# TtesseractT/Synthetic-Audio-Detection

Measured on AMD Instinct MI355X. Metric: 4s@32kHz segments/sec end-to-end (mel+ResNet+ensemble), 1/2/4/8 MI355X, higher is better.
Workload: dtype bf16; 1 GPU; end-to-end inference: B int16 4 s segments resident in HBM -> mel front end -> ResNet-18@512x512 -> 6 binary heads -> merge (+RCCL all-gather of logits); heads=6, distinct_backbones=1, micro_batch=2048, parallelism=dp1, frontend_overlapped=True

## Files before the change

### synthetic-audio-detection_amd/csrc/api.hip

```cpp
#include <math.h>
#include <stdlib.h>
#include <string.h>

#include <mutex>
#include <string>
#include <vector>

#include "common.hpp"
#include "kernels.hpp"

namespace sad {

static thread_local std::string g_err;
void set_error(const std::string& msg) { g_err = msg; }

struct ConvSpec {
  int cin, cout, k, stride, pad;
};
static std::vector<ConvSpec> resnet18_specs() {
  std::vector<ConvSpec> v;
  v.push_back({3, 64, 7, 2, 3});
  int inp = 64;
  const int planes[4] = {64, 128, 256, 512};
  for (int li = 0; li < 4; ++li) {
// ... 334 lines not shown
}

extern "C" int sad_profile_end(int32_t variant, double* total_ms, int64_t* launches, double* flops) {
  SAD_REQUIRE(total_ms && launches && flops, "null outputs");
  std::lock_guard<std::mutex> lk(g_prof_mu);
  g_prof_on = false;
  double ms = 0.0, fl = 0.0;
  int64_t n = 0;
  for (auto& r : g_prof) {
    if (variant == 0 || r.variant == variant) {
      SAD_CHECK_HIP(hipEventSynchronize(r.e1));
      float t = 0.f;
      SAD_CHECK_HIP(hipEventElapsedTime(&t, r.e0, r.e1));
      ms += t;
      fl += r.flops;
      n += r.kernels;
    }
    (void)hipEventDestroy(r.e0);
    (void)hipEventDestroy(r.e1);
  }
  g_prof.clear();
  *total_ms = ms;
  *launches = n;
  *flops = fl;
  return SAD_OK;
}

static int run_blocks(const sad_backbone_plan* p, size_t b0, size_t b1, int64_t n, void** in, void** alt, void* tmp,
                      int& H, int& C, hipStream_t s, float* pool_out = nullptr, bool* pooled = nullptr) {
  int rc;
  void* bufA = *in;
  void* bufB = *alt;
  void* bufT = tmp;
  const int64_t mb = n;
  {
    for (size_t bi = b0; bi < b1; ++bi) {
      const DevBlock& blk = p->blocks[bi];
      const int Ho = H / blk.stride;
      if (p->dtype == SAD_BF16 && blk.stride == 1 && blk.cout == 64 && C == 64 && blk.cin == 64 && H % 16 == 0 &&
          l1_fused()) {
        L1BlockArgs f{};
        f.x = (const u16*)bufA;
        f.out = (u16*)bufB;
        f.N = (int)mb;
        f.H = f.W = H;
        f.w1 = (const u16*)blk.w1;
        f.w1_ld = 9 * 64;
        f.b1 = blk.b1;
        f.w2 = (const u16*)blk.w2;
        f.w2_ld = 9 * 64 + blk.cin_sc;
        f.b2 = blk.b2;
        if ((rc = timed_l1block(f, s, 2.0 * 2.0 * mb * H * H * 64 * 576.0))) return rc;
        std::swap(bufA, bufB);
        continue;
      }
      BlockConvArgs a{};
      a.in0 = bufA;
      a.in0_pstride = C;
      a.N = (int)mb;
      a.H = a.W = H;
      a.Cin = C;
      a.KH = a.KW = 3;
      a.stride = blk.stride;
      a.pad = 1;
      a.wt = blk.w1;
      a.bias = blk.b1;
      a.out = bufT;
      a.out_pstride = blk.cout;
      a.Ho = a.Wo = Ho;
      a.Cout = blk.cout;
      a.relu = 1;
      a.M = mb * Ho * Ho;
      if ((rc = timed_block_conv(a, p->dtype, s, 2.0 * a.M * a.Cout * 9.0 * C))) return rc;
      BlockConvArgs b2 = a;
      b2.in0 = bufT;
      b2.in0_pstride = blk.cout;
      b2.H = b2.W = Ho;
      b2.Cin = blk.cout;
      b2.stride = 1;
      b2.wt_ld = 9 * blk.cout + blk.cin_sc;
      if ((p->dtype == SAD_BF16 || p->dtype == SAD_BF16X3) && blk.stride == 1 && Ho % 16 == 0 &&
          (blk.cout <= 64 || (blk.cout <= 128 && layer2_halo() && !(p->dtype == SAD_BF16 && layer2_v31()) &&
                            !(p->dtype == SAD_BF16X3 && x3_layer2_v31())))) {
        b2.res = bufA;
        b2.res_pstride = C;
      } else {
        b2.in1 = bufA;
        b2.in1_pstride = C;
        b2.H1 = b2.W1 = H;
        b2.Cin1 = C;
        b2.ss1 = blk.stride;
      }
      b2.wt = blk.w2;
      b2.bias = blk.b2;
      b2.out = bufB;
      if (pool_out && bi + 1 == b1 && block_conv_can_pool(b2, p->dtype)) {
        b2.pool_out = pool_out;
        b2.out = nullptr;
        *pooled = true;
      }
      const double fl2 = 2.0 * b2.M * b2.Cout * (9.0 * blk.cout + (blk.stride != 1 ? (double)C : 0.0));
      if ((rc = timed_block_conv(b2, p->dtype, s, fl2))) return rc;
      std::swap(bufA, bufB);
      H = Ho;
      C = blk.cout;
    }
  }
  *in = bufA;
  *alt = bufB;
  return SAD_OK;
}

static int front_sub_batch(int dtype) {
  static int v = [] {
    const char* e = getenv("SAD_FRONT_MB");
    return e ? atoi(e) : -1;
  }();
  if (v >= 0) return v;
  return dtype == SAD_BF16 && l1_fused() ? 256 : dtype == SAD_BF16X3 ? 64 : 32;
}

static int run_chunk(const sad_backbone_plan* p, const float* map, const float* img, int64_t mb, float* feats,
                     void* layer4_out, char* ws, hipStream_t s, const float* img3 = nullptr) {
  const size_t ab = act_bytes(p, mb);
  void* bufA = ws;
  void* bufB = ws + ab;
  void* bufT = ws + 2 * ab;
  void* bufD = ws + 3 * ab;
  int rc;
  int H = 128, C = 64;
  bool pooled = false;
  if (p->block_path) {
    const size_t es = p->dtype == SAD_BF16 ? 2 : 4;
    const int64_t f = front_sub_batch(p->dtype) > 0 ? std::min<int64_t>(front_sub_batch(p->dtype), mb) : mb;
    const size_t l1_elems = 128 * 128 * 64;
    for (int64_t i = 0; i < mb; i += f) {
      const int64_t n = std::min(f, mb - i);
      void* a0 = bufA;
      void* a1 = bufB;
      StemArgs st{map ? map + i * p->mh * p->mw : nullptr, img ? img + i * 512 * 512 : nullptr, p->mh, p->mw,
                  p->stem_w, p->stem_b, a0, n, img3 ? img3 + i * 3 * 512 * 512 : nullptr, p->stem_w3};
      if ((rc = launch_stem(st, p->dtype, s))) return rc;
      H = 128;
      C = 64;
      if ((rc = run_blocks(p, 0, 1, n, &a0, &a1, bufT, H, C, s))) return rc;
      void* slot = (char*)bufD + (size_t)i * l1_elems * es;
      void* dst = slot;
      void* src = a0;
      if ((rc = run_blocks(p, 1, 2, n, &src, &dst, bufT, H, C, s))) return rc;
      if (src != slot) {
        set_error("internal: layer1 output not in its bufD slot");
        return SAD_ERR_STATE;
      }
    }
    void* a0 = bufD;
    void* a1 = bufA;
    if ((rc = run_blocks(p, 2, p->blocks.size(), mb, &a0, &a1, bufB, H, C, s, layer4_out ? nullptr : feats,
                         &pooled)))
      return rc;
    bufA = a0;
  } else {
    StemArgs st{map, img, p->mh, p->mw, p->stem_w, p->stem_b, bufA, mb, img3, p->stem_w3};
    if ((rc = launch_stem(st, p->dtype, s))) return rc;
  }
  size_t ci = 0;
  for (int li = 0; li < 4 && !p->block_path; ++li) {
// ... 403 lines not shown
```

### synthetic-audio-detection_amd/csrc/block.hip

```cpp
#include <stdio.h>
#include <stdlib.h>

#include <algorithm>
#include <atomic>
#include <type_traits>
#include <vector>

#include "common.hpp"
#include "igemm.hpp"
#include "kernels.hpp"

#ifndef SAD_STAMPS
#define SAD_STAMPS 0
#endif

namespace sad {

#define SAD_STAMP(slot)                                                                          \
  do {                                                                                           \
    if constexpr (SAD_STAMPS) {                                                                  \
      if (stamp_on) {                                                                            \
        __builtin_amdgcn_sched_barrier(0);                                                       \
        uint64_t t_;                                                                             \
        asm volatile("s_memtime %0\n\ts_waitcnt lgkmcnt(0)" : "=s"(t_)::"memory");              \
// ... 526 lines not shown
  g = std::max<int64_t>(n_tc, g / n_tc * n_tc);
  const int64_t nk = (int64_t)a.KH * a.KW * a.Cin * sizeof(T) / 128 + (a.in1 ? a.Cin1 * sizeof(T) / 128 : 0);
  SAD_REQUIRE(a.M + BP < (1ll << 31) && (tiles_p / (g / n_tc) + 1) * nk < (1ll << 31),
              "block conv: too many pixels for one launch (lower the micro-batch)");
  if constexpr (ST_OK) {
    if (a.st_part) {
      *a.st_rows = (int)(g / n_tc);
      hipLaunchKernelGGL((block_conv_kernel<T, WC, WP, TC, TP, S, OCC, false, X3, true>), dim3((unsigned)g),
                         dim3(64 * WC * WP), smem, s, a);
      SAD_CHECK_HIP(hipGetLastError());
      return SAD_OK;
    }
  }
  if constexpr (RES_OK) {
    if (a.res) {
      hipLaunchKernelGGL((block_conv_kernel<T, WC, WP, TC, TP, S, OCC, true, X3, false, X4>), dim3((unsigned)g),
                         dim3(64 * WC * WP), smem, s, a);
      SAD_CHECK_HIP(hipGetLastError());
      return SAD_OK;
    }
  }
  hipLaunchKernelGGL((block_conv_kernel<T, WC, WP, TC, TP, S, OCC, false, X3, false, X4>), dim3((unsigned)g),
                     dim3(64 * WC * WP),
                     smem, s, a);
  SAD_CHECK_HIP(hipGetLastError());
  return SAD_OK;
}

template <typename T, bool X3 = false>
static int launch_block_v(const BlockConvArgs& a, int v, hipStream_t s) {
  switch (v) {
    case 9: return launch_block_t<T, 1, 4, 4, 4, 2, 2, false, X3>(a, s);
    case 10: return launch_block_t<T, 2, 2, 4, 4, 2, 2, false, X3>(a, s);
    case 11: return launch_block_t<T, 1, 4, 4, 4, 3, 1, false, X3>(a, s);
    case 12: return launch_block_t<T, 2, 2, 4, 4, 3, 1, false, X3>(a, s);
    case 13: return launch_block_t<T, 2, 4, 8, 4, 2, 1, true, X3, sizeof(T) == 2 && !X3>(a, s);
    case 14: return launch_block_t<T, 2, 4, 4, 4, 2, 1, false, X3>(a, s);
    case 15: return launch_block_t<T, 2, 4, 4, 4, 3, 1, false, X3, sizeof(T) == 2 && !X3>(a, s);
    case 16: return launch_block_t<T, 1, 8, 4, 4, 2, 1, false, X3>(a, s);
    case 17: return launch_block_t<T, 2, 2, 8, 4, 2, 1, false, X3>(a, s);
    case 18: return launch_block_t<T, 2, 2, 4, 8, 2, 1, false, X3>(a, s);
    case 19: return launch_block_t<T, 1, 8, 8, 4, 2, 1, false, X3>(a, s);
  }
  set_error("unknown block-conv variant");
  return SAD_ERR_ARG;
}
static int launch_block_x4(const BlockConvArgs& a, int v, hipStream_t s) {
  switch (v) {
    case 9: return launch_block_t<u16, 1, 4, 4, 4, 2, 2, false, true, false, true>(a, s);
    case 13: return launch_block_t<u16, 2, 4, 8, 4, 2, 1, true, true, false, true>(a, s);
    case 15: return launch_block_t<u16, 2, 4, 4, 4, 3, 1, false, true, false, true>(a, s);
  }
  set_error("four-product split-bf16 convs run on the implicit-GEMM variants 9, 13, 15");
  return SAD_ERR_ARG;
}

int launch_halo_v(const BlockConvArgs& a, int v, hipStream_t s, bool x3 = false);
int launch_halo256(const BlockConvArgs& a, hipStream_t s, bool x3);
int launch_halo256r(const BlockConvArgs& a, hipStream_t s, bool x3);
bool halo256_ok(const BlockConvArgs& a);
int launch_halo_rw(const BlockConvArgs& a, hipStream_t s);
int launch_l2conv(const BlockConvArgs& a, hipStream_t s, bool x3 = false);
int launch_halo256s2(const BlockConvArgs& a, hipStream_t s);
bool halo256s2_ok(const BlockConvArgs& a);
int launch_halo_rw_x3(const BlockConvArgs& a, hipStream_t s);
int launch_l2s2conv(const BlockConvArgs& a, hipStream_t s);
int launch_halo256rs2(const BlockConvArgs& a, hipStream_t s, bool x3);
bool halo256rs2_ok(const BlockConvArgs& a);

static bool halo_ok(const BlockConvArgs& a, int dtype) {
  return (dtype == SAD_BF16 || dtype == SAD_BF16X3) && a.KH == 3 && a.KW == 3 && a.stride == 1 && a.pad == 1 &&
         !a.in1 && a.Cin % (dtype == SAD_BF16X3 ? 32 : 64) == 0 && a.Cout % 64 == 0 && a.W % 16 == 0 &&
         a.H % 16 == 0;
}
bool layer2_v31() {
  static const bool v = [] {
    const char* e = getenv("SAD_L2_V31");
    return e ? atoi(e) != 0 : false;
  }();
  return v;
}
static bool halo31_ok(const BlockConvArgs& a) {
  return a.KH == 3 && a.KW == 3 && a.stride == 1 && a.pad == 1 && a.Cout % 128 == 0 && a.H % 16 == 0 &&
         a.W % 16 == 0 && a.Ho == a.H && a.Wo == a.W && !a.res && !a.st_part && a.Cin % 64 == 0 &&
         (!a.in1 || a.Cin1 % 64 == 0) && (!a.pool_out || (a.H == 16 && a.W == 16 && a.Cout % 256 == 0));
}
bool x3_layer2_v31() {
  static const bool v = [] {
    const char* e = getenv("SAD_X3_L2_V31");
    return e ? atoi(e) != 0 : true;
  }();
  return v;
}
static bool l2_rw() {
  static const bool v = [] {
    const char* e = getenv("SAD_L2_RW");
    return e ? atoi(e) != 0 : true;
  }();
  return v;
}
static bool l2_ds_rw() {
  static const bool v = [] {
    const char* e = getenv("SAD_L2_DS_RW");
    return e ? atoi(e) != 0 : true;
  }();
  return v;
}
static bool l2conv_ds_ok(const BlockConvArgs& a) {
  return a.KH == 3 && a.KW == 3 && a.stride == 1 && a.pad == 1 && a.Cin == 128 && a.Cout == 128 && a.H % 16 == 0 &&
         a.W % 16 == 0 && a.Ho == a.H && a.Wo == a.W && a.in1 && a.Cin1 == 64 && a.ss1 == 2 && a.H1 == 2 * a.H &&
         a.W1 == 2 * a.W && !a.res && !a.pool_out && !a.st_part;
}
static int s2_patch() {
  static const int v = [] {
    const char* e = getenv("SAD_S2_PATCH");
    return e ? atoi(e) : 2;
  }();
  return v;
}
static int x3_s2_variant() {
  static const int v = [] {
    const char* e = getenv("SAD_X3_S2");
    return e ? atoi(e) : 44;
  }();
  return v;
}
static bool l2s2_rw() {
  static const bool v = [] {
    const char* e = getenv("SAD_L2S2_RW");
    return e ? atoi(e) != 0 : true;
  }();
  return v;
}
static bool l2s2_ok(const BlockConvArgs& a) {
  return a.KH == 3 && a.KW == 3 && a.stride == 2 && a.pad == 1 && a.Cin == 64 && a.Cout == 128 && a.Ho % 16 == 0 &&
         a.Wo % 16 == 0 && a.H == 2 * a.Ho && a.W == 2 * a.Wo && !a.in1 && !a.res && !a.pool_out;
}
bool layer2_halo() {
  static const bool v = [] {
    const char* e = getenv("SAD_L2_HALO");
    return e ? atoi(e) != 0 : true;
  }();
  return v;
}
static int c128_variant() {
  static const int v = [] {
    const char* e = getenv("SAD_C128_VARIANT");
    return e ? atoi(e) : 15;
  }();
  return v;
}
static int halo_c128_variant() {
  static const int v = [] {
    const char* e = getenv("SAD_HALO_C128");
    return e ? atoi(e) : 20;
  }();
  return v;
}
static int x3_l1_variant() {
  static const int v = [] {
    const char* e = getenv("SAD_X3_L1");
    return e ? atoi(e) : 42;
  }();
  return v;
}
static bool x3_rw() {
  static const bool v = [] {
    const char* e = getenv("SAD_X3_RW");
    return e ? atoi(e) != 0 : true;
  }();
  return v;
}
static int x3_halo256_variant() {
  static const int v = [] {
    const char* e = getenv("SAD_X3_HALO256");
    return e ? atoi(e) : 30;
  }();
  return v;
}
static int halo256_mode() {
  static const int v = [] {
    const char* e = getenv("SAD_HALO256");
    return e ? atoi(e) : 2;
  }();
  return v;
}
static int block_device_cus() {
  static int cus[64] = {};
  int dev = 0;
  if (hipGetDevice(&dev) != hipSuccess || dev < 0 || dev >= 64) return 256;
  if (!cus[dev]) {
    int c = 0;
    if (hipDeviceGetAttribute(&c, hipDeviceAttributeMultiprocessorCount, dev) != hipSuccess || c <= 0) c = 256;
    cus[dev] = c;
  }
  return cus[dev];
}
int default_block_variant(const BlockConvArgs& a, int dtype) {
  if (dtype == SAD_BF16X3) {
    if (halo_ok(a, dtype) && a.Cin == 64 && a.Cout == 64 && x3_l1_variant() == 42) return 42;
    if (halo_ok(a, dtype) && a.Cin == 64 && a.Cout == 64 && x3_rw()) return 26;
    if (x3_layer2_v31() && a.Cout == 128 && halo31_ok(a)) return 31;
    if (halo256_mode() != 0 && (halo256_mode() == 1 || x3_halo256_variant() == 30) && halo256_ok(a)) return 30;
    if (halo256_mode() == 2 && x3_halo256_variant() == 31 && a.Cout % 256 == 0 && halo31_ok(a)) return 31;
    if (x3_s2_variant() == 44 && halo256rs2_ok(a) && a.Cout % 256 == 0) return 44;
    return halo_ok(a, dtype) && a.Cout <= 128 ? 20 : (a.Cout % 256 == 0 ? 13 : (a.Cout % 128 == 0 ? c128_variant() : 9));
  }
  if (halo_ok(a, dtype) && a.Cin == 64 && a.Cout == 64) return 25;
  if (dtype == SAD_BF16 && l2_rw() && halo_ok(a, dtype) && a.Cin == 128 && a.Cout == 128 && !a.st_part) return 41;
  if (dtype == SAD_BF16 && l2_ds_rw() && l2conv_ds_ok(a)) return 41;
  if (dtype == SAD_BF16 && layer2_v31() && a.Cout == 128 && halo31_ok(a)) return 31;
  if (halo_ok(a, dtype) && (a.res || (a.Cout <= 128 && layer2_halo())))
    return a.Cout == 128 && !a.res && halo_c128_variant() == 22 ? 22 : 20;
  if (dtype == SAD_BF16 && halo256_mode() != 0 && halo256_ok(a)) return halo256_mode() == 2 ? 31 : 30;
  if (dtype == SAD_BF16 && l2s2_rw() && l2s2_ok(a)) return 43;
  if (dtype == SAD_BF16 && s2_patch() == 2 && halo256rs2_ok(a)) return 44;
  if (dtype == SAD_BF16 && s2_patch() == 1 && halo256s2_ok(a)) return 32;
  return gemm_block_variant(a);
}
int gemm_block_variant(const BlockConvArgs& a) {
  if (a.Cout % 256 == 0)
    return a.res || (a.M + 255) / 256 * (a.Cout / 256) >= block_device_cus() ? 13 : 15;
  return a.Cout % 128 == 0 ? c128_variant() : 9;
}
static int pool_tile(int v) {
  switch (v) {
    case 13: case 14: case 15: case 30: case 31: return 256;
    case 16: return 512;
  }
  return 0;
}
bool block_conv_can_pool(const BlockConvArgs& a, int dtype) {
  const int v = default_block_variant(a, dtype);
  const int bp = pool_tile(v);
  return bp > 0 && a.Ho * a.Wo == bp && !a.res && a.M % bp == 0 && (v != 31 || a.Cout % 256 == 0);
}
static bool variant_fits(int v, int cout) {
  if (v == 26 || v == 42) return cout == 64;
  if (v == 30) return cout % 256 == 0;
  if (v == 31 || v == 32 || v == 44) return cout % 128 == 0;
  const int bc[] = {0, 0, 0, 0, 0, 0, 0, 0, 0, 64, 128, 64, 128, 256, 128, 128, 64, 256, 128, 128};
  if (v == 20 || v == 21) return cout % 64 == 0;
  if (v == 22) return cout % 128 == 0;
  if (v == 25) return cout == 64;
  if (v == 41 || v == 43) return cout == 128;
  return v >= 9 && v <= 19 && cout % bc[v] == 0;
}

#if SAD_STAMPS
constexpr size_t kStampWords = SAD_CLOCK_BASE + 4 * SAD_CLOCK_WGS;
static bool stamp_this_launch(int which) {
  static const int every = [] {
    const char* e = getenv("SAD_STAMP_EVERY");
    return e ? std::max(1, atoi(e)) : 1;
  }();
  static long count[2] = {0, 0};
  return count[which]++ % every == every - 1;
}
static int stamp_report(const BlockConvArgs& a, hipStream_t s) {
  std::vector<uint64_t> h(kStampWords);
  SAD_CHECK_HIP(hipStreamSynchronize(s));
  SAD_CHECK_HIP(hipMemcpy(h.data(), a.stamps, h.size() * 8, hipMemcpyDeviceToHost));
  {
    std::vector<double> clk, dur, xcd[8];
    uint64_t r0 = ~0ull, r0max = 0, r1min = ~0ull, r1 = 0;
    for (int g = 0; g < SAD_CLOCK_WGS; ++g) {
      const uint64_t* c = &h[SAD_CLOCK_BASE + 4 * g];
      if (!c[0] || !c[2] || c[3] <= c[1]) continue;
      clk.push_back((double)(c[2] - c[0]) / (double)(c[3] - c[1]) * 100.0);
      xcd[g % 8].push_back(clk.back());
      dur.push_back((double)(c[3] - c[1]) / 100.0);
      r0 = std::min(r0, c[1]); r0max = std::max(r0max, c[1]);
      r1min = std::min(r1min, c[3]); r1 = std::max(r1, c[3]);
    }
    if (!clk.empty()) {
      std::sort(clk.begin(), clk.end());
      std::sort(dur.begin(), dur.end());
      fprintf(stderr, "clock M=%lld Cout=%d: %zu workgroups, in-kernel clock median %.0f MHz (min %.0f, max %.0f); "
              "span %.1f us, workgroup time median %.1f us (min %.1f, max %.1f), starts spread %.1f us, "
              "ends spread %.1f us\n", (long long)a.M, a.Cout, clk.size(), clk[clk.size() / 2], clk.front(),
              clk.back(), (r1 - r0) / 100.0, dur[dur.size() / 2], dur.front(), dur.back(), (r0max - r0) / 100.0,
              (r1 - r1min) / 100.0);
      fprintf(stderr, "clock per XCD (median MHz):");
      for (auto& x : xcd) {
        if (x.empty()) continue;
        std::sort(x.begin(), x.end());
        fprintf(stderr, " %.0f", x[x.size() / 2]);
      }
      fprintf(stderr, "\n");
    }
  }
  for (int w = 0; w < 2; ++w) {
    double ph[4] = {0, 0, 0, 0};
    int n = 0;
    for (int g = a.N <= 64 ? 1 : 8; g + 1 < 1024; ++g) {
      const uint64_t* t = &h[w * 4096 + g * 4];
      const uint64_t t0n = h[w * 4096 + (g + 1) * 4];
      if (!t[0] || !t[3] || !t0n || t0n < t[3]) break;
      ph[0] += (double)(t[1] - t[0]);
      ph[1] += (double)(t[2] - t[1]);
      ph[2] += (double)(t[3] - t[2]);
      ph[3] += (double)(t0n - t[3]);
      ++n;
    }
    if (n)
      fprintf(stderr, "stamps M=%lld Cout=%d K=%d wave %d: %d steps, cycles/step phases 0-1 %.0f | 1-2 %.0f | "
              "2-3 %.0f | 3-next %.0f | total %.0f\n", (long long)a.M, a.Cout, a.KH * a.KW * a.Cin, w, n,
              ph[0] / n, ph[1] / n, ph[2] / n, ph[3] / n, (ph[0] + ph[1] + ph[2] + ph[3]) / n);
  }
  return SAD_OK;
}
#endif

static thread_local int64_t g_block_conv_kernels = 0;
int64_t block_conv_kernel_launches() { return g_block_conv_kernels; }

int launch_block_conv(const BlockConvArgs& a_in, int dtype, hipStream_t s, int variant) {
  SAD_REQUIRE(dtype == SAD_F32 || dtype == SAD_BF16 || dtype == SAD_BF16X3, "dtype");
// ... 150 lines not shown
```

### synthetic-audio-detection_amd/csrc/halo256r.hip

```cpp
#include "common.hpp"
#include "igemm.hpp"
#include "kernels.hpp"
#include "rwconv.hpp"

namespace sad {

namespace h31 {
constexpr int NW = 8, TC = 2;
constexpr int TW = 16, TH = 16, PW = TW + 2, PR = PW * (TH + 2);
constexpr int NDP = (PR + 7) / 8;
constexpr int SCR = PW * TH;
constexpr int NDS = SCR / 8;
constexpr int PATCH = NDP * 1024;
constexpr int ROWB = PW * 128;
constexpr int SMEM = 2 * PATCH;
constexpr int BAD = 0x7FFFFFF0;
constexpr uint64_t KEY = 0xd92dad912240ull;
static_assert(SMEM <= 160 * 1024, "LDS budget");
}

__device__ __forceinline__ int h31_key(int px) { return (int)((h31::KEY >> (3 * px)) & 7); }

typedef unsigned int h31_v4 __attribute__((ext_vector_type(4)));
typedef __bf16 h31_bf2 __attribute__((ext_vector_type(2)));
typedef float h31_f2 __attribute__((ext_vector_type(2)));
__device__ __forceinline__ uint32_t h31_pk(float lo, float hi) {
  return __builtin_bit_cast(uint32_t, __builtin_convertvector((h31_f2){lo, hi}, h31_bf2));
}
__device__ __forceinline__ uint32_t h31_relu2(uint32_t x) {
  uint32_t r;
  asm("v_pk_max_i16 %0, %1, 0" : "=v"(r) : "v"(x));
  return r;
}

template <int BC, bool POOL, bool X3 = false>
__global__ __launch_bounds__(512, 1) void halo256r_kernel(BlockConvArgs a) {
  using namespace h31;
  constexpr int NCG = BC / 32, NPG = NW / NCG, TP = 16 / NPG;
  static_assert(NCG * NPG == NW && (!POOL || NPG == 1), "wave split");
  extern __shared__ __attribute__((aligned(16))) char smem[];
  const int tid = threadIdx.x, lane = tid & 63;
  const int wave = __builtin_amdgcn_readfirstlane(tid >> 6);
  const int fr = lane & 15, fg = lane >> 4;
  const int n_tc = a.Cout / BC;
  const int w = xcd_remap(blockIdx.x, gridDim.x);
  const int tc = w % n_tc;
  const int gp = gridDim.x / n_tc, wi = w / n_tc;
  const int tiles_x = a.W / TW, tiles_img = tiles_x * (a.H / TH);
  const int tiles_p = a.N * tiles_img;
  const int tp_begin = (int)((int64_t)wi * tiles_p / gp), tp_end = (int)((int64_t)(wi + 1) * tiles_p / gp);
  const int c0 = tc * BC;
  if (tp_begin >= tp_end) return;
  const int cgrp = wave % NCG, pgrp = wave / NCG;
  const int cw = c0 + cgrp * 16 * TC;
  const int r0w = pgrp * TP;

  const int cinb = a.Cin * 2;
  const int nc0 = cinb / 128;
  const int nk1 = a.in1 ? a.Cin1 * 2 / 128 : 0;
  const int nch = nc0 + nk1;

  const __amdgpu_buffer_rsrc_t r0 =
      __builtin_amdgcn_make_buffer_rsrc((void*)a.in0, (short)0, (int)a.in0_bytes, 0x00020000);
  const __amdgpu_buffer_rsrc_t r1 =
      __builtin_amdgcn_make_buffer_rsrc((void*)(a.in1 ? a.in1 : a.in0), (short)0, (int)a.in1_bytes, 0x00020000);
  const __amdgpu_buffer_rsrc_t rw =
      __builtin_amdgcn_make_buffer_rsrc((void*)a.wt, (short)0, (int)a.wt_bytes, 0x00020000);
  const int ps0 = (int)a.in0_pstride * 2, ps1 = (int)a.in1_pstride * 2;
  const unsigned lds0 = (unsigned)(uintptr_t)(__attribute__((address_space(3))) char*)smem;
  const int lrow = lane >> 3;
  const int ab = a.ablate;

  const int wrow = a.wt_ld * 2;
  const int wlane = (cw + fr) * wrow + fg * 16;
  auto load_w = [&](int kb, h31_v4 (&wv)[TC][2]) __attribute__((always_inline)) {
#pragma unroll
    for (int i = 0; i < TC; ++i)
#pragma unroll
      for (int h = 0; h < 2; ++h)
        wv[i][h] = __builtin_amdgcn_raw_buffer_load_b128(rw, wlane + i * 16 * wrow + kb + h * 64, 0, 0);
  };
  auto kb_of = [&](int c, int tap) __attribute__((always_inline)) {
    return c < nc0 ? tap * cinb + c * 128 : 9 * cinb + (c - nc0) * 128;
  };

  struct TileO {
    int b, oy0, ox0;
    bool ok;
  };
  auto tile_o = [&](int t) __attribute__((always_inline)) {
    const int tt = __builtin_amdgcn_readfirstlane(t);
    const int b = tt / tiles_img, rem = tt - b * tiles_img;
    const int ty = rem / tiles_x;
    return TileO{b, ty * TH, (rem - ty * tiles_x) * TW, tt < tp_end};
  };
  auto issue_patch = [&](const TileO& to, int c, int buf, int k_only) __attribute__((always_inline)) {
    if (!to.ok) return;
    const int b = to.b, oy0 = to.oy0, ox0 = to.ox0;
    int lr;
    asm volatile("v_mov_b32 %0, %1" : "=v"(lr) : "v"(lrow));
    const unsigned dst = lds0 + buf * PATCH;
    if (c < nc0) {
      const int base = ((b * a.H + oy0 - 1) * a.W + ox0 - 1) * ps0 + c * 128;
#pragma unroll
      for (int k = 0; k < (NDP + NW - 1) / NW; ++k) {
        const int q = wave + NW * k;
        if ((k_only < 0 || k == k_only) && q < NDP) {
          const int s = 8 * q + lr, py = s / PW, px = s - py * PW;
          const int iy = oy0 - 1 + py, ix = ox0 - 1 + px;
          const int off = (s < PR && (unsigned)iy < (unsigned)a.H && (unsigned)ix < (unsigned)a.W)
                              ? base + (py * a.W + px) * ps0 + (((lane & 7) ^ h31_key(px)) << 4)
                              : BAD;
          dma16_m0(r0, off, dst + q * 1024);
        }
      }
    } else {
      const int base = ((b * a.H1 + oy0 * a.ss1) * a.W1 + ox0 * a.ss1) * ps1 + (c - nc0) * 128;
#pragma unroll
      for (int k = 0; k < (NDS + NW - 1) / NW; ++k) {
        const int q = wave + NW * k;
        if ((k_only < 0 || k == k_only) && q < NDS) {
          const int s = 8 * q + lr, ty = s / PW, tx = s - ty * PW;
          const int off = tx < TW ? base + (ty * a.W1 + tx) * (a.ss1 * ps1) + (((lane & 7) ^ h31_key(tx)) << 4)
                                  : BAD;
          dma16_m0(r1, off, dst + q * 1024);
        }
      }
    }
  };

  issue_patch(tile_o(tp_begin), 0, 0, -1);
  f32x4 biasv[TC];
#pragma unroll
  for (int i = 0; i < TC; ++i) biasv[i] = *(const f32x4*)(a.bias + cw + i * 16 + fg * 4);
  h31_v4 wcur[TC][2], wnxt[TC][2];
  load_w(0, wnxt);

  f32x4 acc[TC][TP];
#pragma unroll
  for (int i = 0; i < TC; ++i)
#pragma unroll
    for (int j = 0; j < TP; ++j) acc[i][j] = biasv[i];

  auto take_w = [&]() __attribute__((always_inline)) {
#pragma unroll
    for (int i = 0; i < TC; ++i)
#pragma unroll
      for (int h = 0; h < 2; ++h) wcur[i][h] = wnxt[i][h];
  };

  auto step = [&](int pbuf, int ky, int kx) __attribute__((always_inline)) {
    const int pbase = pbuf * PATCH + (ky + r0w) * ROWB;
    const int o0 = (kx + fr) * 128 + ((fg ^ h31_key(kx + fr)) << 4);
    const int o1 = (kx + fr) * 128 + (((fg + 4) ^ h31_key(kx + fr)) << 4);
    const char* pb0 = smem + pbase + o0;
    const char* pb1 = smem + pbase + o1;
    auto half = [&](auto hc) __attribute__((always_inline)) {
      constexpr int h = decltype(hc)::value;
      constexpr int NM = X3 && h == 0 ? 2 : 1;
      const char* pb = h ? pb1 : pb0;
      uint4 bf[TP];
#pragma unroll
      for (int j = 0; j < TP; ++j) bf[j] = *(const uint4*)(pb + j * ROWB);
#pragma unroll
      for (int j = 0; j < TP; ++j)
#pragma unroll
        for (int m = 0; m < NM; ++m)
#pragma unroll
          for (int i = 0; i < TC; ++i)
            mfma_chunk<u16>(__builtin_bit_cast(uint4, wcur[i][X3 ? m : h]), bf[j], acc[i][j]);
      __builtin_amdgcn_sched_group_barrier(0x100, 4, 0);
#pragma unroll
      for (int j = 0; j < TP - 4; ++j) {
        __builtin_amdgcn_sched_group_barrier(0x008, NM * TC, 0);
        __builtin_amdgcn_sched_group_barrier(0x100, 1, 0);
      }
      __builtin_amdgcn_sched_group_barrier(0x008, 4 * NM * TC, 0);
    };
    half(std::integral_constant<int, 0>{});
    half(std::integral_constant<int, 1>{});
  };

  auto epilogue = [&](int t) __attribute__((always_inline)) {
    const int b = t / tiles_img, rem = t - b * tiles_img;
    const int oy0 = (rem / tiles_x) * TH, ox0 = (rem - (rem / tiles_x) * tiles_x) * TW;
    if constexpr (POOL) {
#pragma unroll
      for (int i = 0; i < TC; ++i) {
        float ps[4];
#pragma unroll
        for (int r = 0; r < 4; ++r) {
          float v = 0.f;
#pragma unroll
          for (int j = 0; j < TP; ++j) v += fmaxf(acc[i][j][r], 0.f);
          ps[r] = row16_sum(v);
        }
        if (fr == 0)
          *(float4*)(a.pool_out + (int64_t)b * a.Cout + cw + i * 16 + fg * 4) =
              make_float4(ps[0] * (1.f / 256), ps[1] * (1.f / 256), ps[2] * (1.f / 256), ps[3] * (1.f / 256));
      }
    } else {
      u16* __restrict__ out = (u16*)a.out;
#pragma unroll
      for (int j = 0; j < TP; j += 2) {
        const int64_t px = (int64_t)(b * a.H + oy0 + r0w + j + (fg & 1)) * a.W + ox0 + fr;
#pragma unroll
        for (int i = 0; i < TC; ++i) {
          if constexpr (X3) {
            float v[2][4];
#pragma unroll
            for (int r = 0; r < 4; ++r) {
              v[0][r] = a.relu ? fmaxf(acc[i][j][r], 0.f) : acc[i][j][r];
              v[1][r] = a.relu ? fmaxf(acc[i][j + 1][r], 0.f) : acc[i][j + 1][r];
            }
            uint32_t qh[4], ql[4];
#pragma unroll
            for (int e = 0; e < 4; ++e) {
              const float x0 = v[e >> 1][2 * (e & 1)], x1 = v[e >> 1][2 * (e & 1) + 1];
              qh[e] = h31_pk(x0, x1);
              ql[e] = h31_pk(x0 - __uint_as_float(qh[e] << 16), x1 - __uint_as_float(qh[e] & 0xFFFF0000u));
            }
#pragma unroll
            for (int e = 0; e < 2; ++e) {
              const auto rh = __builtin_amdgcn_permlane16_swap(qh[e], qh[e + 2], false, false);
              qh[e] = rh[0];
              qh[e + 2] = rh[1];
              const auto rl = __builtin_amdgcn_permlane16_swap(ql[e], ql[e + 2], false, false);
              ql[e] = rl[0];
              ql[e + 2] = rl[1];
            }
            u16* op = out + px * a.out_pstride + 2 * cw + i * 16 + (fg >> 1) * 8;
            *(uint4*)op = make_uint4(qh[0], qh[1], qh[2], qh[3]);
            *(uint4*)(op + 32) = make_uint4(ql[0], ql[1], ql[2], ql[3]);
            continue;
          }
          const int co = cw + i * 16 + (fg >> 1) * 8;
          uint32_t q[4] = {h31_pk(acc[i][j][0], acc[i][j][1]), h31_pk(acc[i][j][2], acc[i][j][3]),
                           h31_pk(acc[i][j + 1][0], acc[i][j + 1][1]), h31_pk(acc[i][j + 1][2], acc[i][j + 1][3])};
          if (a.relu)
#pragma unroll
            for (int e = 0; e < 4; ++e) q[e] = h31_relu2(q[e]);
#pragma unroll
          for (int e = 0; e < 2; ++e) {
            const auto r = __builtin_amdgcn_permlane16_swap(q[e], q[e + 2], false, false);
            q[e] = r[0];
            q[e + 2] = r[1];
          }
          if (ab & 128) {
            asm volatile("" ::"v"(q[0]), "v"(q[1]), "v"(q[2]), "v"(q[3]));
          } else {
            *(uint4*)(out + px * a.out_pstride + co) = make_uint4(q[0], q[1], q[2], q[3]);
          }
        }
      }
    }
#pragma unroll
    for (int i = 0; i < TC; ++i)
#pragma unroll
      for (int j = 0; j < TP; ++j) acc[i][j] = biasv[i];
  };

  int u = 0;
  bool post_epi = false;
  for (int t = tp_begin; t < tp_end; ++t) {
    for (int c = 0; c < nch; ++c) {
      const bool sc = c >= nc0;
      const int nsteps = sc ? 1 : 9;
      const int nt = c + 1 < nch ? t : t + 1, ncn = c + 1 < nch ? c + 1 : 0;
      const TileO nto = tile_o(nt);
      const int pbuf = u & 1;
      for (int tap = 0; tap < nsteps; ++tap) {
        if (tap == 0) {
          if (post_epi)
            asm volatile("s_waitcnt vmcnt(%0)" ::"n"(POOL ? 0 : (X3 ? 2 : 1) * TC * TP / 2) : "memory");
          else
            asm volatile("s_waitcnt vmcnt(0)" ::: "memory");
          post_epi = false;
          __builtin_amdgcn_s_barrier();
          asm volatile("" ::: "memory");
        }
        take_w();
        if (!(ab & 1)) {
          const int kbn = tap + 1 < nsteps ? kb_of(c, tap + 1) : kb_of(ncn, 0);
          if (!(ab & 4)) load_w(kbn, wnxt);
          if (ab & 2) {
          } else if (sc) {
            issue_patch(nto, ncn, pbuf ^ 1, -1);
          } else if (tap >= 1 && tap <= 6) {
            issue_patch(nto, ncn, pbuf ^ 1, tap - 1);
          }
        }
        const int ky = sc ? 0 : tap / 3, kx = sc ? 0 : tap - 3 * (tap / 3);
        step(pbuf, ky, kx);
      }
      ++u;
    }
    if (!(ab & 8)) epilogue(t);
    post_epi = true;
  }
  asm volatile("s_waitcnt vmcnt(0)" ::: "memory");
}

template <int BC, bool POOL, bool X3>
static int launch_halo256r_t(const BlockConvArgs& a, hipStream_t s) {
  using namespace h31;
  static bool attr = false;
  if (!attr) {
    (void)hipFuncSetAttribute((const void*)halo256r_kernel<BC, POOL, X3>,
                              hipFuncAttributeMaxDynamicSharedMemorySize, SMEM);
    attr = true;
  }
  const int n_tc = a.Cout / BC;
  const int64_t tiles_p = (int64_t)a.N * (a.H / TH) * (a.W / TW);
  int64_t g = std::min<int64_t>(tiles_p * n_tc, 256);
  g = std::max<int64_t>(n_tc, g / n_tc * n_tc);
  hipLaunchKernelGGL((halo256r_kernel<BC, POOL, X3>), dim3((unsigned)g), dim3(512), SMEM, s, a);
  SAD_CHECK_HIP(hipGetLastError());
  return SAD_OK;
}

int launch_halo256r(const BlockConvArgs& a, hipStream_t s, bool x3) {
  SAD_REQUIRE(a.KH == 3 && a.KW == 3 && a.stride == 1 && a.pad == 1, "variant 31: 3x3, stride 1, pad 1");
  SAD_REQUIRE(!a.res && !a.st_part, "variant 31: no epilogue residual / fused statistics (shortcut as in1)");
  SAD_REQUIRE(a.Cout % 128 == 0, "variant 31: Cout must be a multiple of 128");
  SAD_REQUIRE(a.H % 16 == 0 && a.W % 16 == 0 && a.Ho == a.H && a.Wo == a.W, "variant 31: image must tile by 16 x 16");
  SAD_REQUIRE((a.Cin * 2) % 128 == 0 && (!a.in1 || (a.Cin1 * 2) % 128 == 0), "variant 31: whole 128-B chunks");
  SAD_REQUIRE(!a.in1 || ((a.Ho - 1) * a.ss1 < a.H1 && (a.Wo - 1) * a.ss1 < a.W1), "variant 31: shortcut source");
  SAD_REQUIRE(a.wt_ld >= 9 * a.Cin + (a.in1 ? a.Cin1 : 0) && (a.wt_ld * 2) % 16 == 0, "variant 31: weight rows");
  SAD_REQUIRE(a.out_pstride % 8 == 0 && a.in0_pstride % 8 == 0 && (!a.in1 || a.in1_pstride % 8 == 0),
              "variant 31: pixel strides");
  SAD_REQUIRE(a.out || a.pool_out, "null output");
  SAD_REQUIRE(a.M == (int64_t)a.N * a.H * a.W, "variant 31: M = N H W");
  if (a.pool_out) {
    SAD_REQUIRE(a.H == 16 && a.W == 16 && a.Cout % 256 == 0,
                "variant 31 fused average pool: a 16 x 16 tile must be one image, Cout % 256");
    return x3 ? launch_halo256r_t<256, true, true>(a, s) : launch_halo256r_t<256, true, false>(a, s);
  }
  if (x3)
    return a.Cout % 256 == 0 ? launch_halo256r_t<256, false, true>(a, s) : launch_halo256r_t<128, false, true>(a, s);
  return a.Cout % 256 == 0 ? launch_halo256r_t<256, false, false>(a, s) : launch_halo256r_t<128, false, false>(a, s);
}

}
```

### synthetic-audio-detection_amd/csrc/kernels.hpp

```cpp
#pragma once
#include <vector>

#include "common.hpp"

namespace sad {

#define SAD_CLOCK_BASE 8192
#define SAD_CLOCK_WGS 4096
#define SAD_CLOCK_STAMP(slot)                                                                      \
  do {                                                                                             \
    if constexpr (SAD_STAMPS) {                                                                    \
      if (a.stamps && wave == 0 && blockIdx.x < SAD_CLOCK_WGS) {                                   \
        const uint64_t t_ = __builtin_amdgcn_s_memtime();                                          \
        const uint64_t r_ = __builtin_amdgcn_s_memrealtime();                                      \
        if (lane == 0) {                                                                           \
          a.stamps[SAD_CLOCK_BASE + 4 * blockIdx.x + 2 * (slot)] = t_;                             \
          a.stamps[SAD_CLOCK_BASE + 4 * blockIdx.x + 2 * (slot) + 1] = r_;                         \
        }                                                                                          \
      }                                                                                            \
    }                                                                                              \
  } while (0)

struct ConvArgs {
  const void* in;
// ... 5 lines not shown
  int64_t res_pstride;
  void* out;
  int64_t out_pstride;
  int Ho, Wo, Cout, KH, KW, stride, pad;
  int relu;
  int64_t M;
  int64_t in_bytes;
  int64_t wt_bytes;
  int groups;
  int64_t in_gstride, wt_gstride, bias_gstride, out_gstride;
};

struct BlockConvArgs {
  const void* in0;
  int64_t in0_pstride;
  int N, H, W, Cin, KH, KW, stride, pad;
  const void* in1;
  int64_t in1_pstride;
  int H1, W1, Cin1, ss1;
  const void* wt;
  int wt_ld;
  const float* bias;
  const void* res;
  int64_t res_pstride;
  void* out;
  int64_t out_pstride;
  int Ho, Wo, Cout, relu;
  int64_t M;
  int64_t in0_bytes, in1_bytes, wt_bytes, res_bytes;
  int64_t out_bytes;
  int ablate;
  float* pool_out;
  uint64_t* stamps;
  float* st_part;
  int* st_rows;
  int x4;
};

struct L1BlockArgs {
  const u16* x;
  u16* out;
  int N, H, W;
  const u16* w1;
  int w1_ld;
  const float* b1;
  const u16* w2;
  int w2_ld;
  const float* b2;
  int64_t x_bytes;
  int ablate;
  uint64_t* stamps;
};
int launch_l1block(const L1BlockArgs& a, hipStream_t s);
int64_t block_conv_kernel_launches();
bool l1_fused();

struct StemArgs {
  const float* map;
  const float* img;
  int mh, mw;
  const void* w;
  const float* bias;
  void* out;
  int64_t B;
  const float* img3;
  const float* w3;
  const u16* img16;
  float* part;
  int x4;
};

int launch_conv(const ConvArgs& a, int dtype, hipStream_t s, int variant = 0);
int default_conv_variant(const ConvArgs& a);
int launch_stem(const StemArgs& a, int dtype, hipStream_t s);
int launch_stem_train(const StemArgs& a, hipStream_t s);
constexpr int STEM_TRAIN_PARTS = 16;
int launch_block_conv(const BlockConvArgs& a, int dtype, hipStream_t s, int variant = 0);
int default_block_variant(const BlockConvArgs& a, int dtype);
int gemm_block_variant(const BlockConvArgs& a);
bool layer2_halo();
bool x3_layer2_v31();
bool layer2_v31();
bool block_conv_can_pool(const BlockConvArgs& a, int dtype);
int launch_col2im(const float* dcol, int64_t N, int H, int W, int C, int k, int stride, int pad, int Ho, int Wo,
                  int accumulate, void* dx, int dtype, hipStream_t s);
int launch_avgpool(const void* in, int64_t B, int hw, int c, float* out, int dtype, hipStream_t s);
int launch_heads_final(const float* y2, int64_t B, int n_heads, const float* w3, const float* b3,
                       float* logits, float* merged, hipStream_t s);

template <typename V>
int upload(void** dst, const std::vector<V>& v) {
  SAD_CHECK_HIP(hipMalloc(dst, v.size() * sizeof(V)));
  SAD_CHECK_HIP(hipMemcpy(*dst, v.data(), v.size() * sizeof(V), hipMemcpyHostToDevice));
  return SAD_OK;
}
void fold_bn(const float* g, const float* beta, const float* mu, const float* var, int c,
             std::vector<double>& scale, std::vector<double>& shift);
int upload_typed(void** dst, const std::vector<double>& v, int dtype, int64_t row_len = 0);
int fold_stem(const float* const* params, int dtype, void** w_out, float** b_out, float** w3_out);

}
```

### synthetic-audio-detection_amd/csrc/resnet.hip

```cpp
#include <math.h>
#include <stdlib.h>

#include <algorithm>
#include <vector>

#include "common.hpp"
#include "kernels.hpp"

using namespace sad;

namespace {

struct ConvW {
  int cin = 0, cout = 0, k = 0;
  void* w = nullptr;
  float* b = nullptr;
  int ld = 0;
};

struct Block {
  int cin, width, cout, stride;
  bool has_ds;
  ConvW c1, c2, c3;
};
// ... 125 lines not shown
        if ((rc = fold_conv(q1, blk.cout, inp, 3, dtype, blk.c1)) ||
            (rc = fold_conv(q2, blk.cout, blk.cout, 3, dtype, blk.c2, qd, inp, !blk.has_ds))) {
          p->blocks.push_back(blk);
          sad_resnet_plan_destroy(p);
          return rc;
        }
        p->max_elems = std::max<int64_t>(p->max_elems, (int64_t)Ho * Ho * blk.cout);
      } else {
        if ((rc = fold_conv(q1, blk.width, inp, 1, dtype, blk.c1)) ||
            (rc = fold_conv(q2, blk.width, blk.width, 3, dtype, blk.c2)) ||
            (rc = fold_conv(q3, blk.cout, blk.width, 1, dtype, blk.c3, qd, inp, false))) {
          p->blocks.push_back(blk);
          sad_resnet_plan_destroy(p);
          return rc;
        }
        p->max_elems = std::max<int64_t>(p->max_elems, (int64_t)H * H * blk.width);
        p->max_elems = std::max<int64_t>(p->max_elems, (int64_t)Ho * Ho * blk.cout);
      }
      p->blocks.push_back(blk);
      inp = blk.cout;
      H = Ho;
    }
  }
  *out = p;
  return SAD_OK;
}

extern "C" int sad_resnet_num_features(const sad_resnet_plan* p, int32_t* n) {
  SAD_REQUIRE(p && n, "null args");
  *n = p->num_features;
  return SAD_OK;
}

static size_t rn_act_bytes(const sad_resnet_plan* p, int64_t mb) {
  const size_t es = p->dtype == SAD_BF16 ? 2 : 4;
  return ((size_t)mb * p->max_elems * es + 255) & ~(size_t)255;
}

extern "C" int sad_resnet_workspace_size(const sad_resnet_plan* p, int64_t mb, size_t* bytes) {
  SAD_REQUIRE(p && bytes && mb > 0, "bad args");
  *bytes = 4 * rn_act_bytes(p, mb);
  return SAD_OK;
}

static int rn_block_conv(const sad_resnet_plan* p, const ConvW& c, const void* x, int64_t n, int H, int stride,
                         const void* sc, int Hs, int sc_cin, int sc_stride, void* y, hipStream_t s,
                         const void* res = nullptr) {
  const int pad = c.k / 2;
  const int Ho = (H + 2 * pad - c.k) / stride + 1;
  BlockConvArgs a{};
  a.in0 = x;
  a.in0_pstride = c.cin;
  a.N = (int)n;
  a.H = a.W = H;
  a.Cin = c.cin;
  a.KH = a.KW = c.k;
  a.stride = stride;
  a.pad = pad;
  if (sc) {
    a.in1 = sc;
    a.in1_pstride = sc_cin;
    a.H1 = a.W1 = Hs;
    a.Cin1 = sc_cin;
    a.ss1 = sc_stride;
  }
  a.wt = c.w;
  a.wt_ld = c.ld;
  a.bias = c.b;
  a.res = res;
  a.res_pstride = c.cout;
  a.out = y;
  a.out_pstride = c.cout;
  a.Ho = a.Wo = Ho;
  a.Cout = c.cout;
  a.relu = 1;
  a.M = n * Ho * Ho;
  a.x4 = p->x4;
  return launch_block_conv(a, p->dtype, s);
}

static bool identity_epilogue(const sad_resnet_plan* p, const Block& b, int Ho) {
  const int dtype = p->dtype;
  if (p->x4 || !(dtype == SAD_BF16 || dtype == SAD_BF16X3) || b.stride != 1 || b.has_ds || Ho % 16 != 0) return false;
  return b.cout <= 64 || (b.cout <= 128 && layer2_halo() && !(dtype == SAD_BF16 && layer2_v31()) &&
                          !(dtype == SAD_BF16X3 && x3_layer2_v31()));
}

static int rn_chunk(const sad_resnet_plan* p, const float* map, const float* img, int64_t n, float* feats, char* ws,
                    hipStream_t s, const float* img3 = nullptr) {
  const size_t ab = rn_act_bytes(p, n);
  void* X = ws;
  void* Y = ws + ab;
  void* T1 = ws + 2 * ab;
  void* T2 = ws + 3 * ab;
  int rc;
  StemArgs st{map, img, p->mh, p->mw, p->stem_w, p->stem_b, X, n, img3, p->stem_w3};
  st.x4 = p->x4;
  if ((rc = launch_stem(st, p->dtype, s))) return rc;
  int H = 128, C = 64;
  for (const Block& b : p->blocks) {
    const int Ho = H / b.stride;
    if (p->block == SAD_BASIC_BLOCK) {
      if (p->dtype == SAD_BF16 && b.stride == 1 && !b.has_ds && b.cin == 64 && b.cout == 64 && H % 16 == 0 &&
          l1_fused()) {
        L1BlockArgs f{};
        f.x = (const u16*)X;
        f.out = (u16*)Y;
        f.N = (int)n;
        f.H = f.W = H;
        f.w1 = (const u16*)b.c1.w;
        f.w1_ld = b.c1.ld;
        f.b1 = b.c1.b;
        f.w2 = (const u16*)b.c2.w;
        f.w2_ld = b.c2.ld;
        f.b2 = b.c2.b;
        if ((rc = launch_l1block(f, s))) return rc;
      } else {
        if ((rc = rn_block_conv(p, b.c1, X, n, H, b.stride, nullptr, 0, 0, 1, T1, s))) return rc;
        if (identity_epilogue(p, b, Ho)) {
          if ((rc = rn_block_conv(p, b.c2, T1, n, Ho, 1, nullptr, 0, 0, 1, Y, s, X))) return rc;
        } else {
          if ((rc = rn_block_conv(p, b.c2, T1, n, Ho, 1, X, H, C, b.stride, Y, s))) return rc;
        }
      }
    } else {
      if ((rc = rn_block_conv(p, b.c1, X, n, H, 1, nullptr, 0, 0, 1, T1, s))) return rc;
      if ((rc = rn_block_conv(p, b.c2, T1, n, H, b.stride, nullptr, 0, 0, 1, T2, s))) return rc;
      if (b.has_ds) {
        if ((rc = rn_block_conv(p, b.c3, T2, n, Ho, 1, X, H, C, b.stride, Y, s))) return rc;
      } else {
        if ((rc = rn_block_conv(p, b.c3, T2, n, Ho, 1, nullptr, 0, 0, 1, Y, s, X))) return rc;
      }
    }
    std::swap(X, Y);
    H = Ho;
    C = b.cout;
  }
  return launch_avgpool(X, n, H * H, C, feats, p->dtype, s);
}

static int rn_run(const sad_resnet_plan* p, const float* map, const float* img, int64_t B, int64_t mb, float* feats,
                  void* ws, size_t ws_bytes, hipStream_t s, const float* img3 = nullptr) {
  SAD_REQUIRE(p && (map || img || img3) && feats && ws, "null args");
  SAD_REQUIRE(B >= 0 && mb > 0, "bad batch");
  size_t need = 0;
  sad_resnet_workspace_size(p, mb, &need);
  if (ws_bytes < need) {
    set_error("workspace too small");
    return SAD_ERR_NOMEM;
  }
  const int64_t plane = img ? 512 * 512 : (int64_t)p->mh * p->mw;
  for (int64_t i = 0; i < B; i += mb) {
    const int64_t n = std::min(mb, B - i);
    int rc = rn_chunk(p, map ? map + i * plane : nullptr, img ? img + i * plane : nullptr, n,
                      feats + i * p->num_features, (char*)ws, s, img3 ? img3 + i * 3 * 512 * 512 : nullptr);
    if (rc) return rc;
  }
  return SAD_OK;
}

extern "C" int sad_resnet_run(const sad_resnet_plan* p, const float* map, int64_t B, int64_t mb, float* feats,
                              void* ws, size_t ws_bytes, void* stream) {
  SAD_REQUIRE(map, "null map");
  return rn_run(p, map, nullptr, B, mb, feats, ws, ws_bytes, (hipStream_t)stream);
}

extern "C" int sad_resnet_run_img(const sad_resnet_plan* p, const float* img, int64_t B, int64_t mb, float* feats,
                                  void* ws, size_t ws_bytes, void* stream) {
// ... 10 lines not shown
```

Measured before the change: 61510 segments/s.

## Fuse identity residual into variant-31 halo conv epilogue instead of K-concatenated shortcut

For stride-1 identity blocks that would select the variant-31 halo kernel, the shortcut is now added as an epilogue residual rather than appended as extra K columns (in1). The kernel gains a RES template path that prefetches residual bf16 values with buffer loads and adds them to the accumulators before the store or the fused pool. This removes the extra GEMM K work of the in1 identity shortcut (Cin more MACs per output), at the cost of epilogue loads, extra registers and more template instantiations.

```diff
diff --git a/synthetic-audio-detection_amd/csrc/api.hip b/synthetic-audio-detection_amd/csrc/api.hip
--- a/synthetic-audio-detection_amd/csrc/api.hip
+++ b/synthetic-audio-detection_amd/csrc/api.hip
@@ -440,6 +440,9 @@
       if ((p->dtype == SAD_BF16 || p->dtype == SAD_BF16X3) && blk.stride == 1 && Ho % 16 == 0 &&
           (blk.cout <= 64 || (blk.cout <= 128 && layer2_halo() && !(p->dtype == SAD_BF16 && layer2_v31()) &&
                             !(p->dtype == SAD_BF16X3 && x3_layer2_v31())))) {
+        b2.res = bufA;
+        b2.res_pstride = C;
+      } else if (blk.stride == 1 && C == blk.cout && block_conv_identity_res31(b2, p->dtype)) {
         b2.res = bufA;
         b2.res_pstride = C;
       } else {
diff --git a/synthetic-audio-detection_amd/csrc/block.hip b/synthetic-audio-detection_amd/csrc/block.hip
--- a/synthetic-audio-detection_amd/csrc/block.hip
+++ b/synthetic-audio-detection_amd/csrc/block.hip
@@ -632,7 +632,7 @@
 }
 static bool halo31_ok(const BlockConvArgs& a) {
   return a.KH == 3 && a.KW == 3 && a.stride == 1 && a.pad == 1 && a.Cout % 128 == 0 && a.H % 16 == 0 &&
-         a.W % 16 == 0 && a.Ho == a.H && a.Wo == a.W && !a.res && !a.st_part && a.Cin % 64 == 0 &&
+         a.W % 16 == 0 && a.Ho == a.H && a.Wo == a.W && !(a.res && a.in1) && !a.st_part && a.Cin % 64 == 0 &&
          (!a.in1 || a.Cin1 % 64 == 0) && (!a.pool_out || (a.H == 16 && a.W == 16 && a.Cout % 256 == 0));
 }
 bool x3_layer2_v31() {
@@ -746,7 +746,23 @@
   }
   return cus[dev];
 }
+bool block_conv_identity_res31(const BlockConvArgs& a, int dtype) {
+  if (dtype != SAD_BF16 || a.in1 || a.res || a.x4 || a.stride != 1 || a.Cin != a.Cout) return false;
+  BlockConvArgs k = a;
+  k.in1 = &k;
+  k.in1_pstride = a.Cout;
+  k.H1 = a.H;
+  k.W1 = a.W;
+  k.Cin1 = a.Cout;
+  k.ss1 = 1;
+  return default_block_variant(k, dtype) == 31;
+}
 int default_block_variant(const BlockConvArgs& a, int dtype) {
+  if (a.res && !a.in1 && halo31_ok(a)) {
+    BlockConvArgs k = a;
+    k.res = nullptr;
+    if (block_conv_identity_res31(k, dtype)) return 31;
+  }
   if (dtype == SAD_BF16X3) {
     if (halo_ok(a, dtype) && a.Cin == 64 && a.Cout == 64 && x3_l1_variant() == 42) return 42;
     if (halo_ok(a, dtype) && a.Cin == 64 && a.Cout == 64 && x3_rw()) return 26;
@@ -783,7 +799,7 @@
 bool block_conv_can_pool(const BlockConvArgs& a, int dtype) {
   const int v = default_block_variant(a, dtype);
   const int bp = pool_tile(v);
-  return bp > 0 && a.Ho * a.Wo == bp && !a.res && a.M % bp == 0 && (v != 31 || a.Cout % 256 == 0);
+  return bp > 0 && a.Ho * a.Wo == bp && (!a.res || v == 31) && a.M % bp == 0 && (v != 31 || a.Cout % 256 == 0);
 }
 static bool variant_fits(int v, int cout) {
   if (v == 26 || v == 42) return cout == 64;
diff --git a/synthetic-audio-detection_amd/csrc/halo256r.hip b/synthetic-audio-detection_amd/csrc/halo256r.hip
--- a/synthetic-audio-detection_amd/csrc/halo256r.hip
+++ b/synthetic-audio-detection_amd/csrc/halo256r.hip
@@ -33,7 +33,7 @@
   return r;
 }
 
-template <int BC, bool POOL, bool X3 = false>
+template <int BC, bool POOL, bool X3 = false, bool RES = false>
 __global__ __launch_bounds__(512, 1) void halo256r_kernel(BlockConvArgs a) {
   using namespace h31;
   constexpr int NCG = BC / 32, NPG = NW / NCG, TP = 16 / NPG;
@@ -181,10 +181,61 @@
     half(std::integral_constant<int, 1>{});
   };
 
+  constexpr int NR = X3 ? 2 : 1;
+  const __amdgpu_buffer_rsrc_t rr = __builtin_amdgcn_make_buffer_rsrc((void*)(RES ? a.res : a.in0), (short)0,
+                                                                      (int)(RES ? a.res_bytes : 0), 0x00020000);
+  const int rps = (int)a.res_pstride * 2, rrow = a.W * rps;
+  auto load_res = [&](int rlane, int j, int i, h31_v4 (&rv)[NR]) __attribute__((always_inline)) {
+#pragma unroll
+    for (int m = 0; m < NR; ++m)
+      rv[m] = __builtin_amdgcn_raw_buffer_load_b128(rr, rlane, j * rrow + (i * 16 + m * 32) * 2, 0);
+  };
+  auto add_res = [&](int i, int j, h31_v4 (&rv)[NR]) __attribute__((always_inline)) {
+#pragma unroll
+    for (int m = 0; m < NR; ++m)
+#pragma unroll
+      for (int e = 0; e < 2; ++e) {
+        const auto r = __builtin_amdgcn_permlane16_swap(rv[m][e], rv[m][e + 2], false, false);
+        rv[m][e] = r[0];
+        rv[m][e + 2] = r[1];
+      }
+#pragma unroll
+    for (int e = 0; e < 4; ++e) {
+      float x0 = __uint_as_float(rv[0][e] << 16), x1 = __uint_as_float(rv[0][e] & 0xFFFF0000u);
+      if constexpr (X3) {
+        x0 += __uint_as_float(rv[1][e] << 16);
+        x1 += __uint_as_float(rv[1][e] & 0xFFFF0000u);
+      }
+      acc[i][j + (e >> 1)][2 * (e & 1)] += x0;
+      acc[i][j + (e >> 1)][2 * (e & 1) + 1] += x1;
+    }
+  };
+
   auto epilogue = [&](int t) __attribute__((always_inline)) {
     const int b = t / tiles_img, rem = t - b * tiles_img;
     const int oy0 = (rem / tiles_x) * TH, ox0 = (rem - (rem / tiles_x) * tiles_x) * TW;
+    auto pix = [&](int j) __attribute__((always_inline)) {
+      return (int64_t)(b * a.H + oy0 + r0w + j + (fg & 1)) * a.W + ox0 + fr;
+    };
+    constexpr int RD = X3 ? TP / 8 : TP / 2;
+    h31_v4 rv[RD][TC][NR];
+    const int rlane = (int)(pix(0) * rps) + ((X3 ? 2 : 1) * cw + (fg >> 1) * 8) * 2;
+    if constexpr (RES)
+#pragma unroll
+      for (int j = 0; j < 2 * RD; j += 2)
+#pragma unroll
+        for (int i = 0; i < TC; ++i) load_res(rlane, j, i, rv[j / 2][i]);
+    auto res_pair = [&](int j) __attribute__((always_inline)) {
+#pragma unroll
+      for (int i = 0; i < TC; ++i) add_res(i, j, rv[(j / 2) % RD][i]);
+      if (j + 2 * RD < TP)
+#pragma unroll
+        for (int i = 0; i < TC; ++i) load_res(rlane, j + 2 * RD, i, rv[(j / 2) % RD][i]);
+    };
     if constexpr (POOL) {
+      if constexpr (RES)
+#pragma unroll
+        for (int j = 0; j < TP; j += 2) res_pair(j);
 #pragma unroll
       for (int i = 0; i < TC; ++i) {
         float ps[4];
@@ -203,7 +254,8 @@
       u16* __restrict__ out = (u16*)a.out;
 #pragma unroll
       for (int j = 0; j < TP; j += 2) {
-        const int64_t px = (int64_t)(b * a.H + oy0 + r0w + j + (fg & 1)) * a.W + ox0 + fr;
+        const int64_t px = pix(j);
+        if constexpr (RES) res_pair(j);
 #pragma unroll
         for (int i = 0; i < TC; ++i) {
           if constexpr (X3) {
@@ -301,12 +353,12 @@
   asm volatile("s_waitcnt vmcnt(0)" ::: "memory");
 }
 
-template <int BC, bool POOL, bool X3>
+template <int BC, bool POOL, bool X3, bool RES>
 static int launch_halo256r_t(const BlockConvArgs& a, hipStream_t s) {
   using namespace h31;
   static bool attr = false;
   if (!attr) {
-    (void)hipFuncSetAttribute((const void*)halo256r_kernel<BC, POOL, X3>,
+    (void)hipFuncSetAttribute((const void*)halo256r_kernel<BC, POOL, X3, RES>,
                               hipFuncAttributeMaxDynamicSharedMemorySize, SMEM);
     attr = true;
   }
@@ -314,14 +366,21 @@
   const int64_t tiles_p = (int64_t)a.N * (a.H / TH) * (a.W / TW);
   int64_t g = std::min<int64_t>(tiles_p * n_tc, 256);
   g = std::max<int64_t>(n_tc, g / n_tc * n_tc);
-  hipLaunchKernelGGL((halo256r_kernel<BC, POOL, X3>), dim3((unsigned)g), dim3(512), SMEM, s, a);
+  hipLaunchKernelGGL((halo256r_kernel<BC, POOL, X3, RES>), dim3((unsigned)g), dim3(512), SMEM, s, a);
   SAD_CHECK_HIP(hipGetLastError());
   return SAD_OK;
 }
+template <int BC, bool POOL, bool X3>
+static int launch_halo256r_r(const BlockConvArgs& a, hipStream_t s) {
+  return a.res ? launch_halo256r_t<BC, POOL, X3, true>(a, s) : launch_halo256r_t<BC, POOL, X3, false>(a, s);
+}
 
 int launch_halo256r(const BlockConvArgs& a, hipStream_t s, bool x3) {
   SAD_REQUIRE(a.KH == 3 && a.KW == 3 && a.stride == 1 && a.pad == 1, "variant 31: 3x3, stride 1, pad 1");
-  SAD_REQUIRE(!a.res && !a.st_part, "variant 31: no epilogue residual / fused statistics (shortcut as in1)");
+  SAD_REQUIRE(!a.st_part, "variant 31: no fused statistics");
+  SAD_REQUIRE(!a.res || !a.in1, "variant 31: one shortcut, the residual (identity) or in1 (K columns)");
+  SAD_REQUIRE(!a.res || (a.res_pstride % 8 == 0 && a.res_pstride >= (x3 ? 2 : 1) * a.Cout),
+              "variant 31: residual pixel stride");
   SAD_REQUIRE(a.Cout % 128 == 0, "variant 31: Cout must be a multiple of 128");
   SAD_REQUIRE(a.H % 16 == 0 && a.W % 16 == 0 && a.Ho == a.H && a.Wo == a.W, "variant 31: image must tile by 16 x 16");
   SAD_REQUIRE((a.Cin * 2) % 128 == 0 && (!a.in1 || (a.Cin1 * 2) % 128 == 0), "variant 31: whole 128-B chunks");
@@ -334,11 +393,11 @@
   if (a.pool_out) {
     SAD_REQUIRE(a.H == 16 && a.W == 16 && a.Cout % 256 == 0,
                 "variant 31 fused average pool: a 16 x 16 tile must be one image, Cout % 256");
-    return x3 ? launch_halo256r_t<256, true, true>(a, s) : launch_halo256r_t<256, true, false>(a, s);
+    return x3 ? launch_halo256r_r<256, true, true>(a, s) : launch_halo256r_r<256, true, false>(a, s);
   }
   if (x3)
-    return a.Cout % 256 == 0 ? launch_halo256r_t<256, false, true>(a, s) : launch_halo256r_t<128, false, true>(a, s);
-  return a.Cout % 256 == 0 ? launch_halo256r_t<256, false, false>(a, s) : launch_halo256r_t<128, false, false>(a, s);
-}
-
-}
+    return a.Cout % 256 == 0 ? launch_halo256r_r<256, false, true>(a, s) : launch_halo256r_r<128, false, true>(a, s);
+  return a.Cout % 256 == 0 ? launch_halo256r_r<256, false, false>(a, s) : launch_halo256r_r<128, false, false>(a, s);
+}
+
+}
diff --git a/synthetic-audio-detection_amd/csrc/kernels.hpp b/synthetic-audio-detection_amd/csrc/kernels.hpp
--- a/synthetic-audio-detection_amd/csrc/kernels.hpp
+++ b/synthetic-audio-detection_amd/csrc/kernels.hpp
@@ -111,6 +111,7 @@
 bool x3_layer2_v31();
 bool layer2_v31();
 bool block_conv_can_pool(const BlockConvArgs& a, int dtype);
+bool block_conv_identity_res31(const BlockConvArgs& a, int dtype);
 int launch_col2im(const float* dcol, int64_t N, int H, int W, int C, int k, int stride, int pad, int Ho, int Wo,
                   int accumulate, void* dx, int dtype, hipStream_t s);
 int launch_avgpool(const void* in, int64_t B, int hw, int c, float* out, int dtype, hipStream_t s);
diff --git a/synthetic-audio-detection_amd/csrc/resnet.hip b/synthetic-audio-detection_amd/csrc/resnet.hip
--- a/synthetic-audio-detection_amd/csrc/resnet.hip
+++ b/synthetic-audio-detection_amd/csrc/resnet.hip
@@ -231,8 +231,17 @@
 static bool identity_epilogue(const sad_resnet_plan* p, const Block& b, int Ho) {
   const int dtype = p->dtype;
   if (p->x4 || !(dtype == SAD_BF16 || dtype == SAD_BF16X3) || b.stride != 1 || b.has_ds || Ho % 16 != 0) return false;
-  return b.cout <= 64 || (b.cout <= 128 && layer2_halo() && !(dtype == SAD_BF16 && layer2_v31()) &&
-                          !(dtype == SAD_BF16X3 && x3_layer2_v31()));
+  if (b.cout <= 64 || (b.cout <= 128 && layer2_halo() && !(dtype == SAD_BF16 && layer2_v31()) &&
+                       !(dtype == SAD_BF16X3 && x3_layer2_v31())))
+    return true;
+  BlockConvArgs a{};
+  a.N = 1;
+  a.H = a.W = a.Ho = a.Wo = Ho;
+  a.Cin = a.Cout = b.cout;
+  a.KH = a.KW = 3;
+  a.stride = a.pad = 1;
+  a.M = (int64_t)Ho * Ho;
+  return block_conv_identity_res31(a, dtype);
 }
 
 static int rn_chunk(const sad_resnet_plan* p, const float* map, const float* img, int64_t n, float* feats, char* ws,
```

After: 61970 segments/s (median of 6 runs). Within noise of the previous version (+0.8%).
